# terraytherapeutics/COATI

Hardware: AMD Instinct MI355X
Metric: molecules/sec (contrastive+AR train step), grande_closed (higher is better)
Workload: dtype bf16; 1 GPU; grande_closed d=256 L=16 nh=16 + E3GNN h=256x5, V=10322, batch 1024/GPU, seq_len 80, 16-atom point clouds, InfoNCE + AR loss, bf16 MFMA operands / fp32 accumulate + fp32 master weights, random-init weights; global_batch=1024, seq_len=80, parallelism=dp1

## Files before the change

### coati_amd/csrc/engine.cpp

```cpp
#include <stdarg.h>
#include <stdio.h>
#include <stdlib.h>
#include <string.h>

#include <algorithm>
#include <string>
#include <vector>

#include "../../include/coati_hip.h"
#include "kernels.h"

#define HIPCHK(x) do { hipError_t _h = (x); if (_h != hipSuccess) { coati_set_error("%s: %s", #x, hipGetErrorString(_h)); return COATI_EHIP; } } while (0)

static thread_local char g_err[512] = "";
void coati_set_error(const char* fmt, ...) {
  va_list ap;
  va_start(ap, fmt);
  vsnprintf(g_err, sizeof(g_err), fmt, ap);
  va_end(ap);
}
extern "C" const char* coati_last_error(void) { return g_err; }
extern "C" int coati_abi_version(void) { return COATI_ABI_VERSION; }

namespace {
// ... 140 lines not shown
  int gtab_rr = 0;
  int wtab_rr = 0;
  float* t_dx = nullptr;
  bf16_t *t_dxa = nullptr, *t_dxb = nullptr, *t_dh4 = nullptr, *t_da = nullptr;
  bool gnn_wg_group = false;
  std::vector<bf16_t*> gl_DO16, gl_du, gl_dP;
  WgradTile* d_gtab = nullptr;
  int gtab_cap = 0, gtab_n = 0;
  long long gtab_sig = -1;
  const void* gtab_ws = nullptr;
  float* nce = nullptr;
  size_t nce_cap = 0;
  float* opt_partial;
  float* ln_partial;
  float* ln_part_x;
  ShadowJob* d_jobs = nullptr;
  int* d_tile_start = nullptr;
  std::vector<ShadowJob> jobs;
  std::vector<int> tile_start;
  int n_job_tiles = 0;
  bool jobs_uploaded = false;
  hipStream_t side = nullptr;
  hipEvent_t ev_fork = nullptr, ev_join = nullptr;
  bool overlap = getenv("COATI_NO_OVERLAP") == nullptr;
  bool gnn_bwd_done = false;
  bool gnn_side_pending = false;
  unsigned long long prof_mask = 0;
  bool prof_paused = false;
  bool prof_keep_overlap = false;
  std::vector<hipEvent_t> ev;
  int ev_used = 0;
  double prof_flops = 0.0;
  double prof_last_bytes = 0.0;
  struct Decode {
    bool active = false;
    int B = 0, Tmax = 0, pos = 0;
    bool ragged = false;
    bf16_t* cache = nullptr;
    float *x = nullptr, *xmid = nullptr, *xn = nullptr, *mean = nullptr, *rstd = nullptr;
    bf16_t *a = nullptr, *qkv = nullptr, *y = nullptr, *hpre = nullptr, *g = nullptr, *af = nullptr;
    int* pos_dev = nullptr;
    long long* tok_dev = nullptr;
    float* inj_dev = nullptr;
    float* logits_dev = nullptr;
    int64_t ldl = 0;
    hipGraphExec_t graph[2] = {nullptr, nullptr};
// ... 698 lines not shown
      WgradArgs a;
      a.A = A; a.lda = lda; a.B = B; a.ldb = ldb; a.M = Mtab; a.N = N; a.K = K; a.dW = e->G + w_off; a.ldw = K; a.dbias = e->G + b_off; a.n_out = 0;
      return wgrad_table_append(tab, a, e->wg_tile);
    };
    for (int l = l_hi - 1; l >= l_lo; --l) {
      const XLayerP& w = e->xl[l];
      COATI_TRY(add(e->w_dqkv[l], 3 * C, p.a1[l], C, 3 * C, C, w.attnw, w.attnb));
      COATI_TRY(add(e->w_dxb[l], C, p.y[l], C, C, C, w.projw, w.projb));
      if (p.tail && l == e->cfg.n_layer_xformer - 1) continue;
      COATI_TRY(add(e->w_dh4[l], 4 * C, p.a2[l], C, 4 * C, C, w.fc1w, w.fc1b));
      COATI_TRY(add(e->w_dxa[l], C, p.g[l], 4 * C, C, 4 * C, w.fc2w, w.fc2b));
    }
    COATI_CHECK_ARG((int)tab.size() <= e->wtab_cap, "wgrad group: table overflow (%zu > %d)", tab.size(), e->wtab_cap);
    slot = e->wtab_rr++ & 3;
    COATI_TRY(upload_table(e, slot, tab, e->d_wtab + (size_t)slot * e->wtab_cap, s, "wgrad group"));
    coati_engine::WTabKey k;
    k.pass = &p; k.lo = l_lo; k.hi = l_hi; k.M = Mtab; k.n = (int)tab.size(); k.sig = sig;
    e->wtab_key[slot] = k;
  }
  ProfScope ps(e, SITE_XF_WGRAD, flops, s, bytes);
  return launch_wgrad_table(e->d_wtab + (size_t)slot * e->wtab_cap, e->wtab_key[slot].n, s, e->wg_tile, M);
}

int xformer_bwd(coati_engine* e, XPass& p, const void* dyf, int dyf_f32, float* dinjection, hipStream_t s, int l_hi = -1, int l_lo = 0,
                const bf16_t* lmh_dlogits = nullptr, bool inputs_only = false) {
  const coati_config& c = e->cfg;
  const int C = c.n_hidden_xformer, L = c.n_layer_xformer, M = p.M;
  if (l_hi < 0) l_hi = L;
  float* DX = e->DX;
  const bool defer = 2 * L + 1 <= COATI_LN_MAX_SLOTS;
  const long long slot_stride = (long long)COATI_LN_PARTIAL_ROWS * 2 * C;
  LnFinishBatch fin;
  memset(&fin, 0, sizeof(fin));
  int nblk = 0;
  auto ln_bwd = [&](const void* dy, int dy_f32, const float* x, const float* mean, const float* rstd, const float* gamma,
                    const float* dres, size_t goff, size_t boff, bf16_t* dx16) -> int {
    if (!defer && inputs_only) return launch_layernorm_bwd(dy, dy_f32, C, x, C, 0, mean, rstd, gamma, dres, DX, dx16, nullptr, nullptr, e->ln_partial, M, C, s);
    if (!defer) return launch_layernorm_bwd(dy, dy_f32, C, x, C, 0, mean, rstd, gamma, dres, DX, dx16, e->G + goff, e->G + boff, e->ln_partial, M, C, s);
    fin.dg_off[fin.n] = (long long)goff;
    fin.db_off[fin.n] = (long long)boff;
    return launch_layernorm_bwd_deferred(dy, dy_f32, C, x, C, 0, mean, rstd, gamma, dres, DX, dx16, e->ln_part_x + (fin.n++) * slot_stride, &nblk, M, C, s);
  };
  auto dgrad_lnbwd = [&](int site, const bf16_t* dY, int K, const bf16_t* WT, const float* x, const float* mean, const float* rstd,
                         const float* gamma, size_t goff, size_t boff, bf16_t* dx16, const bf16_t* chainW = nullptr,
                         bf16_t* chainC = nullptr, bool has_dres = true) -> int {
    if (!defer || c.use_fp8) return 0;
    GemmArgs a;
    memset(&a, 0, sizeof(a));
    a.A = dY; a.lda = K; a.B = WT; a.ldb = K; a.M = M; a.N = C; a.K = K; a.C = DX; a.ldc = C; a.aux_in = has_dres ? DX : nullptr; a.ld_aux = C; a.aux_out = dx16;
    a.lnb_x = x; a.lnb_ldx = C; a.lnb_mean = mean; a.lnb_rstd = rstd; a.lnb_gamma = gamma;
    if (chainW != nullptr && dx16 != nullptr) { a.chain_W = chainW; a.chain_ldw = C; a.chain_C = chainC; a.chain_ldc = C; }
    int nwg = 0;
    if (!lnbwd_rows_supported(a, &nwg) || nwg > COATI_LN_PARTIAL_ROWS) return 0;
    a.lnb_partial = e->ln_part_x + fin.n * slot_stride;
    fin.dg_off[fin.n] = (long long)goff;
    fin.db_off[fin.n] = (long long)boff;
    fin.nblk[fin.n] = nwg;
    ++fin.n;
    ProfScope ps(e, site, 2.0 * M * C * K + (a.chain_W ? 2.0 * M * C * C : 0.0), s,
                 (double)M * K * 2 + (double)C * K * 2 + (double)M * C * (4 + (has_dres ? 4 : 0) + 4 + (dx16 ? 2 : 0)) + (a.chain_W ? (double)M * C * 2 + (double)C * C * 2 : 0.0));
    const int rc = gemm_rows(a, 0, EPI_LNBWD, s);
    return rc == COATI_OK ? 1 : rc;
  };
  const bool grp = e->wg_group && M >= 4096 && !inputs_only;
  const bool wg_each = !grp && !inputs_only;
  COATI_CHECK_ARG(!inputs_only || (!p.tail && !c.use_fp8 && dinjection != nullptr), "xformer_bwd: the inputs-only backward serves a full bf16 pass with an injection");
  if (l_hi == L && p.tail) {
    ProfScope ps(e, SITE_XF_TAIL, 0, s, (double)p.B * C * ((dyf_f32 ? 4 : 2) + 4 + 4 + 2));
    COATI_TRY(launch_layernorm_bwd(dyf, dyf_f32, C, p.t_xL, C, 0, p.t_meanf, p.t_rstdf, e->P + e->lnfw, nullptr, e->t_dx, e->t_dxa, e->G + e->lnfw, e->G + e->lnfb, e->ln_partial, p.B, C, s));
  } else if (l_hi == L) {
    int lnf_fused = 0;
    if (lmh_dlogits != nullptr) {
      lnf_fused = dgrad_lnbwd(SITE_LMHEAD_DGRAD, lmh_dlogits, e->Vpad, e->S + e->lmheadT, p.x[L], p.meanf, p.rstdf, e->P + e->lnfw, e->lnfw, e->lnfb,
                              grp ? e->w_dxa[L - 1] : e->DX16, nullptr, nullptr, false);
      if (lnf_fused < 0) return lnf_fused;
      if (!lnf_fused) COATI_TRY(gemm(e, SITE_LMHEAD_DGRAD, lmh_dlogits, 0, e->Vpad, e->S + e->lmheadT, e->Vpad, M, C, e->Vpad, e->da, C, nullptr, EPI_BF16, nullptr, nullptr, 0, s));
    }
    if (!lnf_fused) {
      ProfScope ps(e, SITE_LN_BWD, 0, s, (double)M * C * ((dyf_f32 ? 4 : 2) + 4 + 4 + 2));
      COATI_TRY(ln_bwd(dyf, dyf_f32, p.x[L], p.meanf, p.rstdf, e->P + e->lnfw, nullptr, e->lnfw, e->lnfb, grp ? e->w_dxa[L - 1] : e->DX16));
    }
  }
  for (int l = l_hi - 1; l >= l_lo; --l) {
    const XLayerP& w = e->xl[l];
    bf16_t* const dxa = grp ? e->w_dxa[l] : e->DX16;
    bf16_t* const dxb = grp ? e->w_dxb[l] : e->DX16;
    bf16_t* const dh4 = grp ? e->w_dh4[l] : e->dh4;
    bf16_t* const dqkv = grp ? e->w_dqkv[l] : e->dqkv;
    bf16_t* const dx_out = l == 0 ? nullptr : (grp ? e->w_dxa[l - 1] : e->DX16);
    int ln2_fused = 0, ln1_fused = 0;
    if (p.tail && l == L - 1) {
      const int Bt = p.B;
      COATI_TRY(gemm(e, SITE_XF_TAIL, e->t_dxa, 0, C, e->S + w.fc2T, C, Bt, 4 * C, C, e->t_dh4, 4 * C, nullptr, EPI_MUL_AUX, p.t_hpre, nullptr, 4 * C, s));
      COATI_TRY(gemm(e, SITE_XF_TAIL, e->t_dh4, 0, 4 * C, e->S + w.fc1T, 4 * C, Bt, C, 4 * C, e->t_da, C, nullptr, EPI_BF16, nullptr, nullptr, 0, s));
      COATI_TRY(wgrad(e, SITE_XF_TAIL, e->t_dh4, 0, 4 * C, p.t_a2, C, Bt, 4 * C, C, e->G + w.fc1w, C, e->G + w.fc1b, 0, s));
      COATI_TRY(wgrad(e, SITE_XF_TAIL, e->t_dxa, 0, C, p.t_g, 4 * C, Bt, C, 4 * C, e->G + w.fc2w, 4 * C, e->G + w.fc2b, 0, s));
      {
        ProfScope ps(e, SITE_XF_TAIL, 0, s, (double)Bt * C * (2 + 4 + 4 + 4 + 2));
        COATI_TRY(launch_layernorm_bwd(e->t_da, 0, C, p.t_xmid, C, 0, p.t_mean2, p.t_rstd2, e->P + w.ln2w, e->t_dx, e->t_dx, e->t_dxb, e->G + w.ln2w, e->G + w.ln2b, e->ln_partial, Bt, C, s));
        if (hipMemsetAsync(DX, 0, (size_t)M * C * sizeof(float), s) != hipSuccess || hipMemsetAsync(dxb, 0, (size_t)M * C * sizeof(bf16_t), s) != hipSuccess) {
          coati_set_error("xformer_bwd: hipMemsetAsync failed");
          return COATI_EHIP;
        }
        COATI_TRY(launch_scatter_rows_add(e->t_dx, e->stop_pos, DX, Bt, p.T, C, s, p.packed ? p.off : nullptr));
        COATI_TRY(launch_scatter_rows_bf16(e->t_dxb, e->stop_pos, dxb, Bt, p.T, C, s, p.packed ? p.off : nullptr));
      }
    } else {
      if (c.use_fp8) {
        GemmArgs a;
        memset(&a, 0, sizeof(a));
        a.C = dh4; a.ldc = 4 * C; a.aux_in = p.hpre[l]; a.ld_aux = 4 * C;
        COATI_TRY(gemm8(e, SITE_FC2_DGRAD, w, 7, dxa, C, M, 4 * C, C, a, EPI_MUL_AUX, s, true));
        memset(&a, 0, sizeof(a));
        a.C = e->da; a.ldc = C;
        COATI_TRY(gemm8(e, SITE_FC1_DGRAD, w, 6, nullptr, 4 * C, M, C, 4 * C, a, EPI_BF16, s));
      } else {
      COATI_TRY(gemm(e, SITE_FC2_DGRAD, dxa, 0, C, e->S + w.fc2T, C, M, 4 * C, C, dh4, 4 * C, nullptr, EPI_MUL_AUX, p.hpre[l], nullptr, 4 * C, s));
      ln2_fused = dgrad_lnbwd(SITE_FC1_DGRAD, dh4, 4 * C, e->S + w.fc1T, p.xmid[l], p.mean2[l], p.rstd2[l], e->P + w.ln2w, w.ln2w, w.ln2b, dxb,
                              e->S + w.projT, e->dyb);
      if (ln2_fused < 0) return ln2_fused;
      if (!ln2_fused) COATI_TRY(gemm(e, SITE_FC1_DGRAD, dh4, 0, 4 * C, e->S + w.fc1T, 4 * C, M, C, 4 * C, e->da, C, nullptr, EPI_BF16, nullptr, nullptr, 0, s));
      }
// ... 15 lines not shown
    COATI_TRY(gemm(e, SITE_PROJ_DGRAD, dxb, 0, C, e->S + w.projT, C, M, C, C, e->dyb, C, nullptr, EPI_BF16, nullptr, nullptr, 0, s));
    }
    if (wg_each) COATI_TRY(wgrad(e, SITE_XF_WGRAD, dxb, 0, C, p.y[l], C, M, C, C, e->G + w.projw, C, e->G + w.projb, 0, s));
    {
      ProfScope ps(e, SITE_ATTN_BWD, 10.0 * M * (double)p.T * C, s, (double)M * 8 * C * 2 + (double)M * c.n_head * 8);
      COATI_TRY(launch_attn_bwd(p.qkv[l], p.y[l], e->dyb, p.lse[l], e->attnD, dqkv, e->cos_t, e->sin_t, p.B, p.T, c.n_head, C / c.n_head, s, p.packed ? p.off : nullptr, p.packed && lpt_on() ? p.ord : nullptr));
    }
    if (c.use_fp8) {
      GemmArgs a;
      memset(&a, 0, sizeof(a));
      a.C = e->da; a.ldc = C;
      COATI_TRY(gemm8(e, SITE_QKV_DGRAD, w, 4, dqkv, 3 * C, M, C, 3 * C, a, EPI_BF16, s));
    } else {
    ln1_fused = dgrad_lnbwd(SITE_QKV_DGRAD, dqkv, 3 * C, e->S + w.attnT, p.x[l], p.mean1[l], p.rstd1[l], e->P + w.ln1w, w.ln1w, w.ln1b, dx_out);
    if (ln1_fused < 0) return ln1_fused;
    if (!ln1_fused) COATI_TRY(gemm(e, SITE_QKV_DGRAD, dqkv, 0, 3 * C, e->S + w.attnT, 3 * C, M, C, 3 * C, e->da, C, nullptr, EPI_BF16, nullptr, nullptr, 0, s));
    }
    if (wg_each) COATI_TRY(wgrad(e, SITE_XF_WGRAD, dqkv, 0, 3 * C, p.a1[l], C, M, 3 * C, C, e->G + w.attnw, C, e->G + w.attnb, 0, s));
    if (!ln1_fused) {
      ProfScope ps(e, SITE_LN_BWD, 0, s, (double)M * C * (2 + 4 + 4 + 4 + 2));
      COATI_TRY(ln_bwd(e->da, 0, p.x[l], p.mean1[l], p.rstd1[l], e->P + w.ln1w, DX, w.ln1w, w.ln1b, dx_out));
    }
  }
  if (grp && l_hi > l_lo) COATI_TRY(xformer_wgrad_group(e, p, l_lo, l_hi, s));
  if (defer && fin.n > 0 && !inputs_only) {
    ProfScope ps(e, SITE_LN_BWD, 0, s, 0.0);
    COATI_TRY(launch_ln_finish_batched(e->ln_part_x, slot_stride, nblk, e->G, fin, C, s));
  }
  if (l_lo > 0) return COATI_OK;
  ProfScope ps(e, SITE_EMBED, 0, s);
  if (inputs_only) return launch_embed_bwd(p.idx, DX, nullptr, dinjection, c.unk_token, p.B, p.T, C, c.n_tok, s, p.packed ? p.off : nullptr, 1);
  if (c.norm_embed) {
    if (dinjection != nullptr) {
      COATI_TRY(launch_embed_bwd(p.idx, DX, nullptr, dinjection, c.unk_token, p.B, p.T, C, c.n_tok, s, p.packed ? p.off : nullptr, 1));
      COATI_TRY(launch_embed_fwd(p.idx, nullptr, nullptr, c.unk_token, DX, p.B, p.T, C, c.n_tok, s, p.packed ? p.row_src : nullptr, M, 2));
    }
    COATI_TRY(launch_layernorm_bwd(DX, 1, C, p.x_emb, C, 0, p.mean0, p.rstd0, e->P + e->emb_lnw, nullptr, p.x[0], nullptr, e->G + e->emb_lnw, e->G + e->emb_lnb,
                                   e->ln_partial, M, C, s));
    return launch_embed_bwd(p.idx, p.x[0], e->G + e->tok_emb, nullptr, c.unk_token, p.B, p.T, C, c.n_tok, s, p.packed ? p.off : nullptr);
  }
  return launch_embed_bwd(p.idx, DX, e->G + e->tok_emb, dinjection, c.unk_token, p.B, p.T, C, c.n_tok, s, p.packed ? p.off : nullptr);
}

int gnn_fwd(coati_engine* e, const long long* atoms, const float* coords, hipStream_t s) {
  const coati_config& c = e->cfg;
  const int H = c.n_hidden_e3nn, Lg = c.n_layer_e3gnn, B = e->B, A = e->A, BA = B * A, Me = BA * A;
  {
// ... 145 lines not shown
  if (grp) COATI_TRY(gnn_wgrad_group(e, s));
  {
    ProfScope ps(e, SITE_GNN_ELEMWISE, 0, s, (double)BA * (H * 4 + H * 4 + 4 + H * 4) + (double)BA * (8 + H * 4) + 30.0 * H * 4);
    COATI_TRY(launch_layernorm_bwd(DH, 1, H, e->g_h32[0], H, 1, nullptr, e->g_rstd[0], nullptr, nullptr, DO, nullptr, nullptr, nullptr, e->ln_partial, BA, H, s));
    if (e->cfg.torch_emb) COATI_TRY(launch_gnn_embed_bwd(e->atoms, nullptr, nullptr, DO, e->G + e->gembw, nullptr, BA, H, s));
    else COATI_TRY(launch_gnn_embed_bwd(e->atoms, e->lut_ix, e->lut_iy, DO, e->G + e->gembw, e->G + e->gembb, BA, H, s));
  }
  return COATI_OK;
}

int head_linear_bwd(coati_engine* e, SgemmBatch& sb, const float* dY, const float* X, int64_t w_off, int64_t b_off, float* dX, int B,
                    int N, int K) {
  const float* W = e->P + w_off;
  COATI_TRY(sgemm_batch_add(sb, dY, 1, N, X, K, 1, e->G + w_off, K, N, K, B, nullptr, 1.f, 1));
  COATI_TRY(sgemm_batch_add(sb, e->ones, 0, 1, dY, N, 1, e->G + b_off, N, 1, N, B, nullptr, 1.f, 1));
  if (dX) COATI_TRY(sgemm_batch_add(sb, dY, N, 1, W, K, 1, dX, K, B, K, N, nullptr, 1.f, 0));
  return COATI_OK;
}

int ensure_side(coati_engine* e) {
  if (e->side) return COATI_OK;
  if (hipStreamCreateWithFlags(&e->side, hipStreamNonBlocking) != hipSuccess ||
      hipEventCreateWithFlags(&e->ev_fork, hipEventDisableTiming) != hipSuccess ||
      hipEventCreateWithFlags(&e->ev_join, hipEventDisableTiming) != hipSuccess) {
    coati_set_error("engine: could not create the side stream");
    return COATI_EHIP;
  }
  return COATI_OK;
}
int fork_side(coati_engine* e, hipStream_t main) {
  COATI_TRY(ensure_side(e));
  if (hipEventRecord(e->ev_fork, main) != hipSuccess || hipStreamWaitEvent(e->side, e->ev_fork, 0) != hipSuccess) {
    coati_set_error("engine: fork failed");
    return COATI_EHIP;
  }
  return COATI_OK;
}
int join_side(coati_engine* e, hipStream_t main) {
  if (hipEventRecord(e->ev_join, e->side) != hipSuccess || hipStreamWaitEvent(main, e->ev_join, 0) != hipSuccess) {
    coati_set_error("engine: join failed");
    return COATI_EHIP;
  }
  return COATI_OK;
}

int point_head_fwd(coati_engine* e, float* out, hipStream_t s) {
  const coati_config& c = e->cfg;
// ... 138 lines not shown
  c.token_mlp = 0;
  c.torch_emb = 0;
  c.old_architecture = 0;
  c.residual = 0;
  COATI_CHECK_SHAPE(c.n_head > 0 && (C == c.n_head * 16 || C == c.n_head * 32), "engine_create_coati2: head size must be 16 or 32 (C=%d, n_head=%d)", C, c.n_head);
  COATI_CHECK_SHAPE(C % 64 == 0 && C <= 1024, "engine_create_coati2: n_hidden_xformer=%d must be a multiple of 64 (<=1024)", C);
  COATI_CHECK_SHAPE(c.n_seq > 0 && c.n_seq <= 256 && c.n_tok > 8, "engine_create_coati2: n_seq must be <= 256");
  COATI_CHECK_SHAPE(c.n_layer_xformer >= 1, "engine_create_coati2: bad layer count");
  coati_engine* e = new coati_engine();
  e->cfg = c;
  e->enc_to_coati = enc_to_coati;
  build_layout(e);
  *out = e;
  return COATI_OK;
}

void coati_engine_destroy(coati_engine* e) {
  if (!e) return;
  for (auto& g : e->dec.graph)
    if (g) hipGraphExecDestroy(g);
  for (auto ev : e->ev) hipEventDestroy(ev);
  if (e->ev_fork) hipEventDestroy(e->ev_fork);
  if (e->ev_join) hipEventDestroy(e->ev_join);
  if (e->side) hipStreamDestroy(e->side);
  for (int i = 0; i < 6; ++i) {
    if (e->h_tab_ev[i]) hipEventDestroy(e->h_tab_ev[i]);
    if (e->h_tab[i]) hipHostFree(e->h_tab[i]);
  }
  delete e;
}

int64_t coati_engine_param_elems(const coati_engine* e) { return e ? e->n_params : 0; }
int64_t coati_engine_trainable_elems(const coati_engine* e) { return e ? e->n_trainable : 0; }
int coati_engine_n_entries(const coati_engine* e) { return e ? (int)e->entries.size() : 0; }
int coati_engine_entry(const coati_engine* e, int i, char* name, int name_cap, int64_t* offset, int32_t* rows, int32_t* cols) {
  COATI_CHECK_ARG(e && i >= 0 && i < (int)e->entries.size() && name && name_cap > 0, "engine_entry: bad argument");
  const Entry& en = e->entries[i];
  snprintf(name, name_cap, "%s", en.name.c_str());
  if (offset) *offset = en.off;
  if (rows) *rows = en.rows;
  if (cols) *cols = en.cols;
  return COATI_OK;
}
int64_t coati_engine_shadow_elems(const coati_engine* e) { return e ? e->n_shadow : 0; }

int coati_engine_reserve(coati_engine* e, int B, int T1, int T2, int A) {
// ... 109 lines not shown
  COATI_CHECK_ARG(!train || (e->G && y_next), "engine_forward: training needs grads and y_next");
  const coati_config& c = e->cfg;
  COATI_CHECK_SHAPE(B > 0 && T1 > 0 && T2 > 0 && A > 0 && T1 <= c.n_seq && T2 <= c.n_seq,
                    "engine_forward: unsupported shape B=%d T1=%d T2=%d A=%d (n_seq=%d)", B, T1, T2, A, c.n_seq);
  COATI_CHECK_SHAPE(rows1 >= 0 && rows2 >= 0 && rows1 <= (int64_t)B * T1 && rows2 <= (int64_t)B * T2 && (rows1 > 0) == (rows2 > 0),
                    "engine_forward: packed row counts %lld / %lld do not fit %d x %d / %d x %d", (long long)rows1, (long long)rows2, B, T1, B, T2);
  hipStream_t s = (hipStream_t)stream;
  const int E = c.n_embd_common;
  COATI_TRY(begin_call(e, "engine_forward", workspace, workspace_bytes, B, T1, T2, A, scal));
  e->p1.idx = reinterpret_cast<const long long*>(raw_tokens);
  e->p2.idx = reinterpret_cast<const long long*>(tokens);
  e->y_next = reinterpret_cast<const long long*>(y_next);
  e->atoms = reinterpret_cast<const long long*>(atoms);
  e->use_point = use_point;
  COATI_TRY(clear_errors(e, scal, s));
  if (train) HIPCHK(hipMemsetAsync(e->G, 0, (size_t)e->n_params * sizeof(float), s));
  if (rows1 > 0) {
    COATI_TRY(pack_pass(e, e->p1, nullptr, rows1, s));
    COATI_TRY(pack_pass(e, e->p2, e->y_next, rows2, s));
  }
  HIPCHK(hipMemsetD32Async((hipDeviceptr_t)e->ones, 0x3f800000, B, s));

  const bool ovl = e->overlap && (e->prof_mask == 0 || e->prof_keep_overlap) && c.use_point_encoder;
  if (!c.use_point_encoder) {
    HIPCHK(hipMemsetAsync(e->h_e3gnn, 0, (size_t)B * E * sizeof(float), s));
  } else if (ovl) {
    COATI_TRY(fork_side(e, s));
    COATI_TRY(gnn_fwd(e, e->atoms, coords, e->side));
  } else {
    COATI_TRY(gnn_fwd(e, e->atoms, coords, s));
  }
  COATI_TRY(launch_find_stop(e->p1.idx, c.stop_token, e->stop_pos, e->err_flag, B, T1, s));
  {
    static const bool no_tail = getenv("COATI_NO_TAIL") != nullptr;
    e->p1.tail = train && !no_tail && !c.use_fp8;
    e->p2.tail = false;
  }
  COATI_TRY(xformer_fwd(e, e->p1, nullptr, s));
  if (ovl) COATI_TRY(join_side(e, s));
  COATI_TRY(point_head_fwd(e, e->h_e3gnn, s));
  COATI_TRY(stop_rows_head_fwd(e, e->h_smiles, s));
  const float *ptok = nullptr, *stok = nullptr;
  SgemmBatch sb;
  COATI_TRY(special_token_add(e, sb, e->h_e3gnn, e->sa, e->ptok, &ptok, s));
  COATI_TRY(special_token_add(e, sb, e->h_smiles, e->sb, e->stok, &stok, s));
  COATI_TRY(launch_sgemm_batch(sb, s));
  COATI_TRY(launch_select_rows(use_point, ptok, stok, e->cliptok, B, E, s));
  if (bad_rows) COATI_TRY(launch_bad_rows(e->p2.idx, bad_rows, B, T2, s));
  if (h_e3gnn) HIPCHK(hipMemcpyAsync(h_e3gnn, e->h_e3gnn, (size_t)B * E * sizeof(float), hipMemcpyDeviceToDevice, s));
  if (h_smiles) HIPCHK(hipMemcpyAsync(h_smiles, e->h_smiles, (size_t)B * E * sizeof(float), hipMemcpyDeviceToDevice, s));
  if (stop_after_heads) {
    e->decoder_pending = true;
    return COATI_OK;
  }
  return forward_decoder_impl(e, s);
}

int coati_engine_forward_decoder(coati_engine* e, void* stream) {
  COATI_CHECK_ARG(e && e->enc_to_coati < 0, "engine_forward_decoder: a COATI2 engine is inference-only (no training step)");
  COATI_CHECK_ARG(e->decoder_pending, "engine_forward_decoder: no forward stopped behind the heads (train | 2)");
  e->decoder_pending = false;
  return forward_decoder_impl(e, (hipStream_t)stream);
}

int coati_engine_encode(coati_engine* e, void* workspace, int64_t workspace_bytes, int B, int T1, int A,
                        const int64_t* raw_tokens, const int64_t* atoms, const float* coords, float* h_smiles,
                        float* h_e3gnn, float* scal, void* stream) {
  COATI_CHECK_ARG(e && e->P && e->S && workspace && scal, "engine_encode: engine not bound / null argument");
  COATI_CHECK_ARG((raw_tokens && h_smiles) || (atoms && coords && h_e3gnn), "engine_encode: nothing to encode");
// ... 225 lines not shown
  COATI_TRY(launch_infonce_rows2(L1, L2, Bg, B, Bg, row0, bad_all, scal + 2, scal + 3, scal + 7, gscale, s));
  {
    SgemmBatch sb;
    COATI_TRY(sgemm_batch_add(sb, L1, 1, Bg, S_loc, E, 1, dC_all, E, Bg, E, B, nullptr, 1.f, 0));
    COATI_TRY(sgemm_batch_add(sb, L2, 1, Bg, C_loc, E, 1, dS_all, E, Bg, E, B, nullptr, 1.f, 0));
    COATI_TRY(launch_sgemm_batch(sb, s));
  }
  {
    SgemmBatch sb;
    COATI_TRY(sgemm_batch_add(sb, L1, Bg, 1, C_all, E, 1, dS_all + (size_t)row0 * E, E, B, E, Bg, nullptr, 1.f, 1));
    COATI_TRY(sgemm_batch_add(sb, L2, Bg, 1, S_all, E, 1, dC_all + (size_t)row0 * E, E, B, E, Bg, nullptr, 1.f, 1));
    COATI_TRY(launch_sgemm_batch(sb, s));
  }
  return COATI_OK;
}

int coati_engine_backward(coati_engine* e, const float* dh_smiles, const float* dh_e3gnn, int stage, void* stream) {
  COATI_CHECK_ARG(e && e->enc_to_coati < 0, "engine_backward: a COATI2 engine is inference-only (no backward)");
  COATI_CHECK_ARG(e->have_fwd && e->G, "engine_backward: no forward / gradient buffer");
  COATI_CHECK_ARG(stage >= 0 && stage <= 5, "engine_backward: bad stage");
  hipStream_t s = (hipStream_t)stream;
  const coati_config& c = e->cfg;
  const int C = c.n_hidden_xformer, H = c.n_hidden_e3nn, E = c.n_embd_common, B = e->B;
  if (stage == 0 || stage == 1) {
    const int M2 = e->p2.M;
    {
      GemmArgs a;
      memset(&a, 0, sizeof(a));
      a.A = e->p2.af; a.lda = C; a.B = e->S + e->lmhead; a.ldb = C; a.M = M2; a.N = c.n_tok; a.K = C;
      a.C = e->dlogits; a.ldc = e->Vpad; a.n_store = e->Vpad; a.lse = e->ce_lse; a.target = e->p2.packed ? e->p2.ypk : e->y_next; a.scal = e->scal;
      ProfScope ps(e, SITE_LMHEAD_DLOGITS, 2.0 * M2 * c.n_tok * C, s, (double)M2 * C * 2 + (double)c.n_tok * C * 2 + (double)M2 * e->Vpad * 2);
      COATI_TRY(gemm_rows(a, 0, EPI_CE_BWD, s));
    }
    COATI_TRY(wgrad(e, SITE_LMHEAD_WGRAD, e->dlogits, 0, e->Vpad, e->p2.af, C, M2, e->Vpad, C, e->G + e->lmhead, C, nullptr, c.n_tok, s));
    HIPCHK(hipMemsetAsync(e->dcliptok, 0, (size_t)B * E * sizeof(float), s));
    COATI_TRY(xformer_bwd(e, e->p2, e->da, 0, e->dcliptok, s, -1, 0, e->dlogits));
    if (dh_e3gnn) HIPCHK(hipMemcpyAsync(e->dhe, dh_e3gnn, (size_t)B * E * sizeof(float), hipMemcpyDeviceToDevice, s));
    else HIPCHK(hipMemsetAsync(e->dhe, 0, (size_t)B * E * sizeof(float), s));
    if (dh_smiles) HIPCHK(hipMemcpyAsync(e->dhs, dh_smiles, (size_t)B * E * sizeof(float), hipMemcpyDeviceToDevice, s));
    else HIPCHK(hipMemsetAsync(e->dhs, 0, (size_t)B * E * sizeof(float), s));
    if (c.token_mlp) {
      HIPCHK(hipMemsetAsync(e->dptok, 0, (size_t)B * E * sizeof(float), s));
      HIPCHK(hipMemsetAsync(e->dstok, 0, (size_t)B * E * sizeof(float), s));
      COATI_TRY(launch_select_rows_bwd(e->use_point, e->dcliptok, e->dptok, e->dstok, B, E, s));
      SgemmBatch sb;
      COATI_TRY(head_linear_bwd(e, sb, e->dptok, e->sa, e->tokw, e->tokb, e->dsa, B, E, E));
      COATI_TRY(head_linear_bwd(e, sb, e->dstok, e->sb, e->tokw, e->tokb, e->dsb, B, E, E));
      COATI_TRY(launch_sgemm_batch(sb, s));
      COATI_TRY(launch_silu_bwd(e->h_e3gnn, e->dsa, e->dhe, (long long)B * E, 1, s));
      COATI_TRY(launch_silu_bwd(e->h_smiles, e->dsb, e->dhs, (long long)B * E, 1, s));
    } else {
      COATI_TRY(launch_select_rows_bwd(e->use_point, e->dcliptok, e->dhe, e->dhs, B, E, s));
    }
    const bool old_arch = c.norm_clips && c.old_architecture;
    if (old_arch) {
      COATI_TRY(launch_layernorm_bwd(e->dhs, 1, E, e->hs_ln, E, 0, e->hs_mean, e->hs_rstd, e->P + e->s2c_lnw, nullptr, e->dhs_ln, nullptr, e->G + e->s2c_lnw, e->G + e->s2c_lnb, e->ln_partial, B, E, s));
      if (c.use_point_encoder)
        COATI_TRY(launch_layernorm_bwd(e->dhe, 1, E, e->hp_ln, E, 0, e->hp_mean, e->hp_rstd, e->P + e->p2c_lnw, nullptr, e->dhp_ln, nullptr, e->G + e->p2c_lnw, e->G + e->p2c_lnb, e->ln_partial, B, E, s));
    }
    {
      SgemmBatch sb;
      if (old_arch) COATI_TRY(head_linear_bwd(e, sb, e->dhs_ln, e->hstop, e->s2c_w, e->s2c_b, e->dhstop, B, E, C));
      else if (c.norm_clips) COATI_TRY(head_linear_bwd(e, sb, e->dhs, e->hs_ln, e->s2c_w, e->s2c_b, e->dhs_ln, B, E, C));
      else COATI_TRY(head_linear_bwd(e, sb, e->dhs, e->hstop, e->s2c_w, e->s2c_b, e->dhstop, B, E, C));
      if (c.use_point_encoder) {
        if (old_arch) COATI_TRY(head_linear_bwd(e, sb, e->dhp_ln, e->hpoint, e->p2c_w, e->p2c_b, e->dhpoint, B, E, H));
        else if (c.norm_clips) COATI_TRY(head_linear_bwd(e, sb, e->dhe, e->hp_ln, e->p2c_w, e->p2c_b, e->dhp_ln, B, E, H));
        else COATI_TRY(head_linear_bwd(e, sb, e->dhe, e->hpoint, e->p2c_w, e->p2c_b, e->dhpoint, B, E, H));
      }
      COATI_TRY(launch_sgemm_batch(sb, s));
    }
    if (c.norm_clips && !old_arch) {
      COATI_TRY(launch_layernorm_bwd(e->dhs_ln, 1, C, e->hstop, C, 0, e->hs_mean, e->hs_rstd, e->P + e->s2c_lnw, nullptr, e->dhstop, nullptr, e->G + e->s2c_lnw, e->G + e->s2c_lnb, e->ln_partial, B, C, s));
      if (c.use_point_encoder)
        COATI_TRY(launch_layernorm_bwd(e->dhp_ln, 1, H, e->hpoint, H, 0, e->hp_mean, e->hp_rstd, e->P + e->p2c_lnw, nullptr, e->dhpoint, nullptr, e->G + e->p2c_lnw, e->G + e->p2c_lnb, e->ln_partial, B, H, s));
    }
  }
  const int Lx = c.n_layer_xformer, Lmid = Lx / 2;
  const bool ovl_bwd = (stage == 0 || stage == 2 || stage == 4) && e->overlap && (e->prof_mask == 0 || e->prof_keep_overlap) && c.use_point_encoder;
  if (stage == 0 || stage == 1) { e->gnn_bwd_done = false; e->gnn_side_pending = false; }
  if (ovl_bwd) {
    COATI_TRY(fork_side(e, s));
    COATI_TRY(gnn_bwd(e, e->dhpoint, e->side));
  }
  if (stage == 0 || stage == 2 || stage == 4) {
    if (e->p1.tail) {
      COATI_TRY(xformer_bwd(e, e->p1, e->dhstop, 1, nullptr, s, Lx, stage == 4 ? Lmid : 0));
    } else {
      float* dxf = reinterpret_cast<float*>(e->dh4);
      HIPCHK(hipMemsetAsync(dxf, 0, (size_t)e->p1.M * C * sizeof(float), s));
      COATI_TRY(launch_scatter_rows_add(e->dhstop, e->stop_pos, dxf, B, e->T1, C, s, e->p1.packed ? e->p1.off : nullptr));
      COATI_TRY(xformer_bwd(e, e->p1, dxf, 1, nullptr, s, Lx, stage == 4 ? Lmid : 0));
    }
  }
  if (stage == 5) COATI_TRY(xformer_bwd(e, e->p1, nullptr, 1, nullptr, s, Lmid, 0));
  if (ovl_bwd && stage == 4) {
    e->gnn_side_pending = true;
  } else if (ovl_bwd || (stage == 5 && e->gnn_side_pending)) {
    COATI_TRY(join_side(e, s));
    e->gnn_bwd_done = true;
    e->gnn_side_pending = false;
  } else if ((stage == 0 || stage == 3) && !e->gnn_bwd_done) {
    if (c.use_point_encoder) COATI_TRY(gnn_bwd(e, e->dhpoint, s));
    e->gnn_bwd_done = true;
  }
  return COATI_OK;
}

int coati_engine_optimizer_step(coati_engine* e, float lr, float beta1, float beta2, float eps, float weight_decay,
                                float max_norm, int step, float* scal, void* stream) {
  COATI_CHECK_ARG(e && e->enc_to_coati < 0, "optimizer_step: a COATI2 engine is inference-only (no optimizer step)");
  COATI_CHECK_ARG(e->P && e->G && e->Mo && e->Vo && scal, "optimizer_step: engine not bound for training");
  COATI_CHECK_ARG(e->have_fwd, "optimizer_step: needs the workspace of a forward call");
  hipStream_t s = (hipStream_t)stream;
  {
    ProfScope ps(e, SITE_OPTIM, 0, s);
    COATI_TRY(launch_grad_sqnorm(e->G, e->n_trainable, e->opt_partial, 1024, scal + 5, max_norm, scal + 8, s));
    COATI_TRY(launch_adamw(e->P, e->G, e->Mo, e->Vo, e->S, e->n_trainable, lr, beta1, beta2, eps, weight_decay, step, scal + 8, 1.f, s, e->err_flag));
  }
  return refresh_shadows_impl(e, stream, true);
}

int coati_engine_set_error_word(coati_engine* e, const int32_t* word_dev, void* stream) {
  COATI_CHECK_ARG(e && word_dev && e->have_ws && e->err_flag && e->scal, "set_error_word: no forward workspace");
  hipStream_t s = (hipStream_t)stream;
  if (hipMemcpyAsync(e->err_flag, word_dev, sizeof(int), hipMemcpyDeviceToDevice, s) != hipSuccess ||
      hipMemcpyAsync(e->scal + 6, word_dev, sizeof(int), hipMemcpyDeviceToDevice, s) != hipSuccess) {
    coati_set_error("set_error_word: copy failed");
// ... 325 lines not shown
```

Before: 48290 molecules/s.

## Overlap head and tail work with wgrad groups across decoder/encoder seams via side stream

```diff
diff --git a/coati_amd/csrc/engine.cpp b/coati_amd/csrc/engine.cpp
--- a/coati_amd/csrc/engine.cpp
+++ b/coati_amd/csrc/engine.cpp
@@ -186,6 +186,7 @@
   bool jobs_uploaded = false;
   hipStream_t side = nullptr;
   hipEvent_t ev_fork = nullptr, ev_join = nullptr;
+  hipEvent_t ev_seam = nullptr;
   bool overlap = getenv("COATI_NO_OVERLAP") == nullptr;
   bool gnn_bwd_done = false;
   bool gnn_side_pending = false;
@@ -930,8 +931,32 @@
   return launch_wgrad_table(e->d_wtab + (size_t)slot * e->wtab_cap, e->wtab_key[slot].n, s, e->wg_tile, M);
 }
 
+int fork_side(coati_engine* e, hipStream_t main);
+
+static bool seam_overlap_on() {
+  static const bool on = getenv("COATI_NO_SEAM_OVERLAP") == nullptr;
+  return on;
+}
+
+static int tail_lnf_bwd(coati_engine* e, XPass& p, const void* dyf, int dyf_f32, hipStream_t s) {
+  const int C = e->cfg.n_hidden_xformer;
+  ProfScope ps(e, SITE_XF_TAIL, 0, s, (double)p.B * C * ((dyf_f32 ? 4 : 2) + 4 + 4 + 2));
+  return launch_layernorm_bwd(dyf, dyf_f32, C, p.t_xL, C, 0, p.t_meanf, p.t_rstdf, e->P + e->lnfw, nullptr, e->t_dx, e->t_dxa, e->G + e->lnfw, e->G + e->lnfb, e->ln_partial, p.B, C, s);
+}
+static int tail_dgrads(coati_engine* e, XPass& p, hipStream_t s) {
+  const int C = e->cfg.n_hidden_xformer, Bt = p.B;
+  const XLayerP& w = e->xl[e->cfg.n_layer_xformer - 1];
+  COATI_TRY(gemm(e, SITE_XF_TAIL, e->t_dxa, 0, C, e->S + w.fc2T, C, Bt, 4 * C, C, e->t_dh4, 4 * C, nullptr, EPI_MUL_AUX, p.t_hpre, nullptr, 4 * C, s));
+  return gemm(e, SITE_XF_TAIL, e->t_dh4, 0, 4 * C, e->S + w.fc1T, 4 * C, Bt, C, 4 * C, e->t_da, C, nullptr, EPI_BF16, nullptr, nullptr, 0, s);
+}
+static int tail_ln2_bwd(coati_engine* e, XPass& p, hipStream_t s) {
+  const int C = e->cfg.n_hidden_xformer, Bt = p.B;
+  const XLayerP& w = e->xl[e->cfg.n_layer_xformer - 1];
+  return launch_layernorm_bwd(e->t_da, 0, C, p.t_xmid, C, 0, p.t_mean2, p.t_rstd2, e->P + w.ln2w, e->t_dx, e->t_dx, e->t_dxb, e->G + w.ln2w, e->G + w.ln2b, e->ln_partial, Bt, C, s);
+}
+
 int xformer_bwd(coati_engine* e, XPass& p, const void* dyf, int dyf_f32, float* dinjection, hipStream_t s, int l_hi = -1, int l_lo = 0,
-                const bf16_t* lmh_dlogits = nullptr, bool inputs_only = false) {
+                const bf16_t* lmh_dlogits = nullptr, bool inputs_only = false, bool* seam = nullptr, bool tail_pre = false) {
   const coati_config& c = e->cfg;
   const int C = c.n_hidden_xformer, L = c.n_layer_xformer, M = p.M;
   if (l_hi < 0) l_hi = L;
@@ -974,8 +999,7 @@
   const bool wg_each = !grp && !inputs_only;
   COATI_CHECK_ARG(!inputs_only || (!p.tail && !c.use_fp8 && dinjection != nullptr), "xformer_bwd: the inputs-only backward serves a full bf16 pass with an injection");
   if (l_hi == L && p.tail) {
-    ProfScope ps(e, SITE_XF_TAIL, 0, s, (double)p.B * C * ((dyf_f32 ? 4 : 2) + 4 + 4 + 2));
-    COATI_TRY(launch_layernorm_bwd(dyf, dyf_f32, C, p.t_xL, C, 0, p.t_meanf, p.t_rstdf, e->P + e->lnfw, nullptr, e->t_dx, e->t_dxa, e->G + e->lnfw, e->G + e->lnfb, e->ln_partial, p.B, C, s));
+    if (!tail_pre) COATI_TRY(tail_lnf_bwd(e, p, dyf, dyf_f32, s));
   } else if (l_hi == L) {
     int lnf_fused = 0;
     if (lmh_dlogits != nullptr) {
@@ -999,13 +1023,12 @@
     int ln2_fused = 0, ln1_fused = 0;
     if (p.tail && l == L - 1) {
       const int Bt = p.B;
-      COATI_TRY(gemm(e, SITE_XF_TAIL, e->t_dxa, 0, C, e->S + w.fc2T, C, Bt, 4 * C, C, e->t_dh4, 4 * C, nullptr, EPI_MUL_AUX, p.t_hpre, nullptr, 4 * C, s));
-      COATI_TRY(gemm(e, SITE_XF_TAIL, e->t_dh4, 0, 4 * C, e->S + w.fc1T, 4 * C, Bt, C, 4 * C, e->t_da, C, nullptr, EPI_BF16, nullptr, nullptr, 0, s));
+      if (!tail_pre) COATI_TRY(tail_dgrads(e, p, s));
       COATI_TRY(wgrad(e, SITE_XF_TAIL, e->t_dh4, 0, 4 * C, p.t_a2, C, Bt, 4 * C, C, e->G + w.fc1w, C, e->G + w.fc1b, 0, s));
       COATI_TRY(wgrad(e, SITE_XF_TAIL, e->t_dxa, 0, C, p.t_g, 4 * C, Bt, C, 4 * C, e->G + w.fc2w, 4 * C, e->G + w.fc2b, 0, s));
       {
         ProfScope ps(e, SITE_XF_TAIL, 0, s, (double)Bt * C * (2 + 4 + 4 + 4 + 2));
-        COATI_TRY(launch_layernorm_bwd(e->t_da, 0, C, p.t_xmid, C, 0, p.t_mean2, p.t_rstd2, e->P + w.ln2w, e->t_dx, e->t_dx, e->t_dxb, e->G + w.ln2w, e->G + w.ln2b, e->ln_partial, Bt, C, s));
+        if (!tail_pre) COATI_TRY(tail_ln2_bwd(e, p, s));
         if (hipMemsetAsync(DX, 0, (size_t)M * C * sizeof(float), s) != hipSuccess || hipMemsetAsync(dxb, 0, (size_t)M * C * sizeof(bf16_t), s) != hipSuccess) {
           coati_set_error("xformer_bwd: hipMemsetAsync failed");
           return COATI_EHIP;
@@ -1067,7 +1090,14 @@
       COATI_TRY(ln_bwd(e->da, 0, p.x[l], p.mean1[l], p.rstd1[l], e->P + w.ln1w, DX, w.ln1w, w.ln1b, dx_out));
     }
   }
-  if (grp && l_hi > l_lo) COATI_TRY(xformer_wgrad_group(e, p, l_lo, l_hi, s));
+  if (grp && l_hi > l_lo) {
+    if (seam != nullptr && l_lo == 0) {
+      COATI_TRY(fork_side(e, s));
+      *seam = true;
+    }
+    COATI_TRY(xformer_wgrad_group(e, p, l_lo, l_hi, s));
+    if (seam != nullptr && *seam) s = e->side;
+  }
   if (defer && fin.n > 0 && !inputs_only) {
     ProfScope ps(e, SITE_LN_BWD, 0, s, 0.0);
     COATI_TRY(launch_ln_finish_batched(e->ln_part_x, slot_stride, nblk, e->G, fin, C, s));
@@ -1259,7 +1289,8 @@
   if (e->side) return COATI_OK;
   if (hipStreamCreateWithFlags(&e->side, hipStreamNonBlocking) != hipSuccess ||
       hipEventCreateWithFlags(&e->ev_fork, hipEventDisableTiming) != hipSuccess ||
-      hipEventCreateWithFlags(&e->ev_join, hipEventDisableTiming) != hipSuccess) {
+      hipEventCreateWithFlags(&e->ev_join, hipEventDisableTiming) != hipSuccess ||
+      hipEventCreateWithFlags(&e->ev_seam, hipEventDisableTiming) != hipSuccess) {
     coati_set_error("engine: could not create the side stream");
     return COATI_EHIP;
   }
@@ -1444,6 +1475,7 @@
   for (auto ev : e->ev) hipEventDestroy(ev);
   if (e->ev_fork) hipEventDestroy(e->ev_fork);
   if (e->ev_join) hipEventDestroy(e->ev_join);
+  if (e->ev_seam) hipEventDestroy(e->ev_seam);
   if (e->side) hipStreamDestroy(e->side);
   for (int i = 0; i < 6; ++i) {
     if (e->h_tab_ev[i]) hipEventDestroy(e->h_tab_ev[i]);
@@ -1599,11 +1631,19 @@
   HIPCHK(hipMemsetD32Async((hipDeviceptr_t)e->ones, 0x3f800000, B, s));
 
   const bool ovl = e->overlap && (e->prof_mask == 0 || e->prof_keep_overlap) && c.use_point_encoder;
+  const bool seam_fwd = ovl && seam_overlap_on() && !c.use_fp8;
+  const float *ptok = nullptr, *stok = nullptr;
   if (!c.use_point_encoder) {
     HIPCHK(hipMemsetAsync(e->h_e3gnn, 0, (size_t)B * E * sizeof(float), s));
   } else if (ovl) {
     COATI_TRY(fork_side(e, s));
     COATI_TRY(gnn_fwd(e, e->atoms, coords, e->side));
+    if (seam_fwd) {
+      SgemmBatch sbp;
+      COATI_TRY(point_head_fwd(e, e->h_e3gnn, e->side));
+      COATI_TRY(special_token_add(e, sbp, e->h_e3gnn, e->sa, e->ptok, &ptok, e->side));
+      COATI_TRY(launch_sgemm_batch(sbp, e->side));
+    }
   } else {
     COATI_TRY(gnn_fwd(e, e->atoms, coords, s));
   }
@@ -1614,14 +1654,14 @@
     e->p2.tail = false;
   }
   COATI_TRY(xformer_fwd(e, e->p1, nullptr, s));
-  if (ovl) COATI_TRY(join_side(e, s));
-  COATI_TRY(point_head_fwd(e, e->h_e3gnn, s));
+  if (ovl && !seam_fwd) COATI_TRY(join_side(e, s));
+  if (!seam_fwd) COATI_TRY(point_head_fwd(e, e->h_e3gnn, s));
   COATI_TRY(stop_rows_head_fwd(e, e->h_smiles, s));
-  const float *ptok = nullptr, *stok = nullptr;
   SgemmBatch sb;
-  COATI_TRY(special_token_add(e, sb, e->h_e3gnn, e->sa, e->ptok, &ptok, s));
+  if (!seam_fwd) COATI_TRY(special_token_add(e, sb, e->h_e3gnn, e->sa, e->ptok, &ptok, s));
   COATI_TRY(special_token_add(e, sb, e->h_smiles, e->sb, e->stok, &stok, s));
   COATI_TRY(launch_sgemm_batch(sb, s));
+  if (seam_fwd) COATI_TRY(join_side(e, s));
   COATI_TRY(launch_select_rows(use_point, ptok, stok, e->cliptok, B, E, s));
   if (bad_rows) COATI_TRY(launch_bad_rows(e->p2.idx, bad_rows, B, T2, s));
   if (h_e3gnn) HIPCHK(hipMemcpyAsync(h_e3gnn, e->h_e3gnn, (size_t)B * E * sizeof(float), hipMemcpyDeviceToDevice, s));
@@ -1893,6 +1933,9 @@
   hipStream_t s = (hipStream_t)stream;
   const coati_config& c = e->cfg;
   const int C = c.n_hidden_xformer, H = c.n_hidden_e3nn, E = c.n_embd_common, B = e->B;
+  const bool seam_ok = seam_overlap_on() && e->overlap && (e->prof_mask == 0 || e->prof_keep_overlap) && !c.use_fp8;
+  bool side_live = false;
+  hipStream_t hs = s;
   if (stage == 0 || stage == 1) {
     const int M2 = e->p2.M;
     {
@@ -1905,29 +1948,30 @@
     }
     COATI_TRY(wgrad(e, SITE_LMHEAD_WGRAD, e->dlogits, 0, e->Vpad, e->p2.af, C, M2, e->Vpad, C, e->G + e->lmhead, C, nullptr, c.n_tok, s));
     HIPCHK(hipMemsetAsync(e->dcliptok, 0, (size_t)B * E * sizeof(float), s));
-    COATI_TRY(xformer_bwd(e, e->p2, e->da, 0, e->dcliptok, s, -1, 0, e->dlogits));
-    if (dh_e3gnn) HIPCHK(hipMemcpyAsync(e->dhe, dh_e3gnn, (size_t)B * E * sizeof(float), hipMemcpyDeviceToDevice, s));
-    else HIPCHK(hipMemsetAsync(e->dhe, 0, (size_t)B * E * sizeof(float), s));
-    if (dh_smiles) HIPCHK(hipMemcpyAsync(e->dhs, dh_smiles, (size_t)B * E * sizeof(float), hipMemcpyDeviceToDevice, s));
-    else HIPCHK(hipMemsetAsync(e->dhs, 0, (size_t)B * E * sizeof(float), s));
+    COATI_TRY(xformer_bwd(e, e->p2, e->da, 0, e->dcliptok, s, -1, 0, e->dlogits, false, seam_ok ? &side_live : nullptr));
+    if (side_live) hs = e->side;
+    if (dh_e3gnn) HIPCHK(hipMemcpyAsync(e->dhe, dh_e3gnn, (size_t)B * E * sizeof(float), hipMemcpyDeviceToDevice, hs));
+    else HIPCHK(hipMemsetAsync(e->dhe, 0, (size_t)B * E * sizeof(float), hs));
+    if (dh_smiles) HIPCHK(hipMemcpyAsync(e->dhs, dh_smiles, (size_t)B * E * sizeof(float), hipMemcpyDeviceToDevice, hs));
+    else HIPCHK(hipMemsetAsync(e->dhs, 0, (size_t)B * E * sizeof(float), hs));
     if (c.token_mlp) {
-      HIPCHK(hipMemsetAsync(e->dptok, 0, (size_t)B * E * sizeof(float), s));
-      HIPCHK(hipMemsetAsync(e->dstok, 0, (size_t)B * E * sizeof(float), s));
-      COATI_TRY(launch_select_rows_bwd(e->use_point, e->dcliptok, e->dptok, e->dstok, B, E, s));
+      HIPCHK(hipMemsetAsync(e->dptok, 0, (size_t)B * E * sizeof(float), hs));
+      HIPCHK(hipMemsetAsync(e->dstok, 0, (size_t)B * E * sizeof(float), hs));
+      COATI_TRY(launch_select_rows_bwd(e->use_point, e->dcliptok, e->dptok, e->dstok, B, E, hs));
       SgemmBatch sb;
       COATI_TRY(head_linear_bwd(e, sb, e->dptok, e->sa, e->tokw, e->tokb, e->dsa, B, E, E));
       COATI_TRY(head_linear_bwd(e, sb, e->dstok, e->sb, e->tokw, e->tokb, e->dsb, B, E, E));
-      COATI_TRY(launch_sgemm_batch(sb, s));
-      COATI_TRY(launch_silu_bwd(e->h_e3gnn, e->dsa, e->dhe, (long long)B * E, 1, s));
-      COATI_TRY(launch_silu_bwd(e->h_smiles, e->dsb, e->dhs, (long long)B * E, 1, s));
+      COATI_TRY(launch_sgemm_batch(sb, hs));
+      COATI_TRY(launch_silu_bwd(e->h_e3gnn, e->dsa, e->dhe, (long long)B * E, 1, hs));
+      COATI_TRY(launch_silu_bwd(e->h_smiles, e->dsb, e->dhs, (long long)B * E, 1, hs));
     } else {
-      COATI_TRY(launch_select_rows_bwd(e->use_point, e->dcliptok, e->dhe, e->dhs, B, E, s));
+      COATI_TRY(launch_select_rows_bwd(e->use_point, e->dcliptok, e->dhe, e->dhs, B, E, hs));
     }
     const bool old_arch = c.norm_clips && c.old_architecture;
     if (old_arch) {
-      COATI_TRY(launch_layernorm_bwd(e->dhs, 1, E, e->hs_ln, E, 0, e->hs_mean, e->hs_rstd, e->P + e->s2c_lnw, nullptr, e->dhs_ln, nullptr, e->G + e->s2c_lnw, e->G + e->s2c_lnb, e->ln_partial, B, E, s));
+      COATI_TRY(launch_layernorm_bwd(e->dhs, 1, E, e->hs_ln, E, 0, e->hs_mean, e->hs_rstd, e->P + e->s2c_lnw, nullptr, e->dhs_ln, nullptr, e->G + e->s2c_lnw, e->G + e->s2c_lnb, e->ln_partial, B, E, hs));
       if (c.use_point_encoder)
-        COATI_TRY(launch_layernorm_bwd(e->dhe, 1, E, e->hp_ln, E, 0, e->hp_mean, e->hp_rstd, e->P + e->p2c_lnw, nullptr, e->dhp_ln, nullptr, e->G + e->p2c_lnw, e->G + e->p2c_lnb, e->ln_partial, B, E, s));
+        COATI_TRY(launch_layernorm_bwd(e->dhe, 1, E, e->hp_ln, E, 0, e->hp_mean, e->hp_rstd, e->P + e->p2c_lnw, nullptr, e->dhp_ln, nullptr, e->G + e->p2c_lnw, e->G + e->p2c_lnb, e->ln_partial, B, E, hs));
     }
     {
       SgemmBatch sb;
@@ -1939,42 +1983,64 @@
         else if (c.norm_clips) COATI_TRY(head_linear_bwd(e, sb, e->dhe, e->hp_ln, e->p2c_w, e->p2c_b, e->dhp_ln, B, E, H));
         else COATI_TRY(head_linear_bwd(e, sb, e->dhe, e->hpoint, e->p2c_w, e->p2c_b, e->dhpoint, B, E, H));
       }
-      COATI_TRY(launch_sgemm_batch(sb, s));
+      COATI_TRY(launch_sgemm_batch(sb, hs));
     }
     if (c.norm_clips && !old_arch) {
-      COATI_TRY(launch_layernorm_bwd(e->dhs_ln, 1, C, e->hstop, C, 0, e->hs_mean, e->hs_rstd, e->P + e->s2c_lnw, nullptr, e->dhstop, nullptr, e->G + e->s2c_lnw, e->G + e->s2c_lnb, e->ln_partial, B, C, s));
+      COATI_TRY(launch_layernorm_bwd(e->dhs_ln, 1, C, e->hstop, C, 0, e->hs_mean, e->hs_rstd, e->P + e->s2c_lnw, nullptr, e->dhstop, nullptr, e->G + e->s2c_lnw, e->G + e->s2c_lnb, e->ln_partial, B, C, hs));
       if (c.use_point_encoder)
-        COATI_TRY(launch_layernorm_bwd(e->dhp_ln, 1, H, e->hpoint, H, 0, e->hp_mean, e->hp_rstd, e->P + e->p2c_lnw, nullptr, e->dhpoint, nullptr, e->G + e->p2c_lnw, e->G + e->p2c_lnb, e->ln_partial, B, H, s));
+        COATI_TRY(launch_layernorm_bwd(e->dhp_ln, 1, H, e->hpoint, H, 0, e->hp_mean, e->hp_rstd, e->P + e->p2c_lnw, nullptr, e->dhpoint, nullptr, e->G + e->p2c_lnw, e->G + e->p2c_lnb, e->ln_partial, B, H, hs));
+    }
+    if (side_live && stage == 1) {
+      COATI_TRY(join_side(e, s));
+      side_live = false;
     }
   }
   const int Lx = c.n_layer_xformer, Lmid = Lx / 2;
   const bool ovl_bwd = (stage == 0 || stage == 2 || stage == 4) && e->overlap && (e->prof_mask == 0 || e->prof_keep_overlap) && c.use_point_encoder;
   if (stage == 0 || stage == 1) { e->gnn_bwd_done = false; e->gnn_side_pending = false; }
-  if (ovl_bwd) {
+  bool tail_pre = false;
+  if (side_live) {
+    if (e->p1.tail) {
+      COATI_TRY(tail_lnf_bwd(e, e->p1, e->dhstop, 1, e->side));
+      COATI_TRY(tail_dgrads(e, e->p1, e->side));
+      COATI_TRY(tail_ln2_bwd(e, e->p1, e->side));
+      tail_pre = true;
+    }
+    if (hipEventRecord(e->ev_seam, e->side) != hipSuccess || hipStreamWaitEvent(s, e->ev_seam, 0) != hipSuccess) {
+      coati_set_error("engine_backward: seam event failed");
+      return COATI_EHIP;
+    }
+    if (ovl_bwd) COATI_TRY(gnn_bwd(e, e->dhpoint, e->side));
+  } else if (ovl_bwd) {
     COATI_TRY(fork_side(e, s));
     COATI_TRY(gnn_bwd(e, e->dhpoint, e->side));
   }
+  bool enc_seam = false;
+  bool* const enc_seam_p = seam_ok ? &enc_seam : nullptr;
   if (stage == 0 || stage == 2 || stage == 4) {
     if (e->p1.tail) {
-      COATI_TRY(xformer_bwd(e, e->p1, e->dhstop, 1, nullptr, s, Lx, stage == 4 ? Lmid : 0));
+      COATI_TRY(xformer_bwd(e, e->p1, e->dhstop, 1, nullptr, s, Lx, stage == 4 ? Lmid : 0, nullptr, false, enc_seam_p, tail_pre));
     } else {
       float* dxf = reinterpret_cast<float*>(e->dh4);
       HIPCHK(hipMemsetAsync(dxf, 0, (size_t)e->p1.M * C * sizeof(float), s));
       COATI_TRY(launch_scatter_rows_add(e->dhstop, e->stop_pos, dxf, B, e->T1, C, s, e->p1.packed ? e->p1.off : nullptr));
-      COATI_TRY(xformer_bwd(e, e->p1, dxf, 1, nullptr, s, Lx, stage == 4 ? Lmid : 0));
-    }
-  }
-  if (stage == 5) COATI_TRY(xformer_bwd(e, e->p1, nullptr, 1, nullptr, s, Lmid, 0));
+      COATI_TRY(xformer_bwd(e, e->p1, dxf, 1, nullptr, s, Lx, stage == 4 ? Lmid : 0, nullptr, false, enc_seam_p));
+    }
+  }
+  if (stage == 5) COATI_TRY(xformer_bwd(e, e->p1, nullptr, 1, nullptr, s, Lmid, 0, nullptr, false, enc_seam_p));
+  bool joined = false;
   if (ovl_bwd && stage == 4) {
     e->gnn_side_pending = true;
   } else if (ovl_bwd || (stage == 5 && e->gnn_side_pending)) {
     COATI_TRY(join_side(e, s));
+    joined = true;
     e->gnn_bwd_done = true;
     e->gnn_side_pending = false;
   } else if ((stage == 0 || stage == 3) && !e->gnn_bwd_done) {
     if (c.use_point_encoder) COATI_TRY(gnn_bwd(e, e->dhpoint, s));
     e->gnn_bwd_done = true;
   }
+  if ((side_live || enc_seam) && !joined) COATI_TRY(join_side(e, s));
   return COATI_OK;
 }
 
```

New measurement: 48760 molecules/s (median of 6 runs). About the same (+1.0%).
